# humanlongevity/tredparse

Hardware: NVIDIA B200
Metric: loci genotyped/sec (higher is better)
Workload: dtype int16 (SW, DPX s16x2) / f64 (likelihood)

## Files before the change

### tredparse_b200/csrc/sw_family.cu

```cuda
#include "internal.cuh"
#include "sw_sweep.cuh"
#include <type_traits>
#include <algorithm>
#include <vector>

namespace {

constexpr int FAM_W2 = 16;
constexpr int FLANK = 18;
constexpr int CLASS_BOTH = 0, CLASS_FWD = 1, CLASS_RC = 2, NCLASS = 3;

struct FamilySmem {
    int8_t prefix[32], suffix[32], repeat[32];
    int Lp, Ls, P, U, clip;
};

struct ClassifyParams {
    const int8_t *rbuf; const int64_t *roff;
    const int32_t *order;
    const int32_t *grp_start;
    const int32_t *chunk_start;
    const int32_t *grp_perm;
    const tredsw_family *families;
    int ngroups;
// ... 76 lines not shown
        Fv[C] = __viaddmax_s16x2(Fv[C], mge2, HOUT);                                          \
    }

constexpr int STAB_PAD = 20;

__host__ __device__ constexpr int strip_units(int P) { return P >= 12 ? 1 : 12 / P; }
__host__ __device__ constexpr int instance_period(int P) { return P == 6 ? 3 : P; }

template <int NC, int PER, bool HAS_IN, bool HAS_OUT, bool HOOK>
__device__ __forceinline__ void strip_pass(const uint32_t *stab, const uint8_t *codes, int lane, int m, int rows2,
                                           const uint32_t *bin, uint32_t *bout, const uint32_t *pot,
                                           uint32_t (&seg)[NC / PER], uint32_t (&mu)[NC / PER], uint32_t mgo2,
                                           uint32_t mge2, uint32_t one) {
    constexpr int K = NC / PER;
    static_assert(K * PER == NC, "strip = whole units");
    constexpr int NG = (NC + 3) / 4;
    uint32_t Hrow[NC], Fv[NC], pend[K];
#pragma unroll
    for (int c = 0; c < NC; ++c) { Hrow[c] = 0; Fv[c] = 0; }
#pragma unroll
    for (int u = 0; u < K; ++u) pend[u] = 0;
    uint32_t hin_prev = 0;
    auto code_at = [&](int j) { return j < m ? (int)codes[j * 32 + lane] : PAIR_GHOST; };
    auto row_of = [&](int code) { return reinterpret_cast<const uint4 *>(stab + code * STAB_PAD); };
    const uint4 *rowA = row_of(code_at(0)), *rowB = row_of(code_at(1));
    uint4 gA = rowA[0], gB = rowB[0];
    uint32_t bA = 0, bB = 0, pA = 0, pB = 0, bA2 = 0, bB2 = 0, pA2 = 0, pB2 = 0;
    const int j1 = min(2, rows2 - 2);
    if (HAS_IN) { bA = bin[lane]; bB = bin[32 + lane]; bA2 = bin[j1 * 32 + lane]; bB2 = bin[(j1 + 1) * 32 + lane]; }
    if (HOOK) { pA = pot[lane]; pB = pot[32 + lane]; pA2 = pot[j1 * 32 + lane]; pB2 = pot[(j1 + 1) * 32 + lane]; }
    int codeA2 = code_at(2), codeB2 = code_at(3);
    for (int j = 0; j < rows2; j += 2) {
        uint32_t hinA = 0, eA = 0, hinB = 0, eB = 0;
        if (HAS_IN) {
            hinA = sw_prmt(bA, 0, 0x4140); eA = sw_prmt(bA, 0, 0x4342);
            hinB = sw_prmt(bB, 0, 0x4140); eB = sw_prmt(bB, 0, 0x4342);
        }
        uint32_t potHA = 0, potEA = 0, potHB = 0, potEB = 0;
        if (HOOK) {
            potHA = sw_prmt(pA, 0, 0x9180); potEA = sw_prmt(pA, 0, 0xb3a2);
            potHB = sw_prmt(pB, 0, 0x9180); potEB = sw_prmt(pB, 0, 0xb3a2);
        }
        const int jn = min(j + 4, rows2 - 2);
        const uint4 *rowA2 = row_of(codeA2), *rowB2 = row_of(codeB2);
        uint32_t bA3 = 0, bB3 = 0, pA3 = 0, pB3 = 0;
        if (HAS_IN) { bA3 = bin[jn * 32 + lane]; bB3 = bin[(jn + 1) * 32 + lane]; }
        if (HOOK) { pA3 = pot[jn * 32 + lane]; pB3 = pot[(jn + 1) * 32 + lane]; }
        const int codeA3 = code_at(j + 4), codeB3 = code_at(j + 5);
        uint32_t sA[NG * 4], sB[NG * 4];
        sA[0] = gA.x; sA[1] = gA.y; sA[2] = gA.z; sA[3] = gA.w;
        sB[0] = gB.x; sB[1] = gB.y; sB[2] = gB.z; sB[3] = gB.w;
        uint32_t hdA = hin_prev, hdB = hinA;
        hin_prev = hinB;
        uint32_t hA = 0, hB = 0;
#pragma unroll
        for (int s = 0; s <= NC; ++s) {
            if ((s & 3) == 0 && s / 4 + 1 < NG) {
                const uint4 a = rowA[s / 4 + 1];
                sA[s + 4] = a.x; sA[s + 5] = a.y; sA[s + 6] = a.z; sA[s + 7] = a.w;
            }
            if (s >= 1 && ((s - 1) & 3) == 0 && (s - 1) / 4 + 1 < NG) {
                const uint4 b = rowB[(s - 1) / 4 + 1];
                sB[s + 3] = b.x; sB[s + 4] = b.y; sB[s + 5] = b.z; sB[s + 6] = b.w;
            }
            if (s == NC - 4 || (NC < 4 && s == 0)) { gA = rowA2[0]; gB = rowB2[0]; }
            if (s < NC) {
                PACKED_CELL(hdA, eA, sA[s], s, hA)
                const int u = s / PER, i = s % PER;
                if (i == 0) pend[u] = hA; else seg[u] = __vimax3_s16x2(seg[u], pend[u], hA);
                if (HOOK && i == PER - 1) {
                    mu[u] = __viaddmax_s16x2(hdA, potHA, mu[u]);
                    mu[u] = __viaddmax_s16x2(eA, potEA, mu[u]);
                }
                if (HAS_OUT && s == NC - 1) bout[j * 32 + lane] = sw_prmt(hA, eA, 0x6420);
            }
            if (s >= 1) {
                PACKED_CELL(hdB, eB, sB[s - 1], s - 1, hB)
                const int u = (s - 1) / PER, i = (s - 1) % PER;
                if (i == PER - 1) seg[u] = __vimax3_s16x2(seg[u], pend[u], hB); else pend[u] = hB;
                if (HOOK && i == PER - 1) {
                    mu[u] = __viaddmax_s16x2(hdB, potHB, mu[u]);
                    mu[u] = __viaddmax_s16x2(eB, potEB, mu[u]);
                }
                if (HAS_OUT && s - 1 == NC - 1) bout[(j + 1) * 32 + lane] = sw_prmt(hB, eB, 0x6420);
            }
        }
        rowA = rowA2; rowB = rowB2; codeA2 = codeA3; codeB2 = codeB3;
        bA = bA2; bB = bB2; bA2 = bA3; bB2 = bB3; pA = pA2; pB = pB2; pA2 = pA3; pB2 = pB3;
    }
}

template <int NC>
__device__ __forceinline__ void suffix_pass(const uint32_t *stab, const uint8_t *codes, int lane, int m, int rows2,
                                            uint32_t *pot, uint32_t &fresh, uint32_t mgo2, uint32_t mge2) {
    constexpr int NG = (NC + 3) / 4;
    uint32_t Grow[NC], Fv[NC];
#pragma unroll
    for (int c = 0; c < NC; ++c) { Grow[c] = 0; Fv[c] = 0; }
    auto code_at = [&](int r) { const int j = rows2 - 1 - r; return (j >= 0 && j < m) ? (int)codes[j * 32 + lane] : PAIR_GHOST; };
    auto row_of = [&](int code) { return reinterpret_cast<const uint4 *>(stab + code * STAB_PAD); };
    uint32_t f0 = 0, f1 = 0;
#define SUFFIX_CELL(GD, E, S, C, GOUT)                                                        \
    {                                                                                         \
        const uint32_t t_ = __vmaxs2(E, Fv[C]);                                               \
        const uint32_t gh_ = __viaddmax_s16x2_relu(t_, mgo2, GD);   \
        GD = Grow[C];                                                                         \
        GOUT = __vadd2(gh_, S);                                                               \
        Grow[C] = GOUT;                                                                       \
        E = __viaddmax_s16x2(E, mge2, gh_);                                                   \
        Fv[C] = __viaddmax_s16x2(Fv[C], mge2, gh_);                                           \
    }
    for (int r = 0; r < rows2; r += 2) {
        const uint4 *rowA = row_of(code_at(r)), *rowB = row_of(code_at(r + 1));
        uint32_t sA[NG * 4], sB[NG * 4];
#pragma unroll
        for (int g = 0; g < NG; ++g) {
            const uint4 a = rowA[g], b = rowB[g];
            sA[4 * g] = a.x; sA[4 * g + 1] = a.y; sA[4 * g + 2] = a.z; sA[4 * g + 3] = a.w;
            sB[4 * g] = b.x; sB[4 * g + 1] = b.y; sB[4 * g + 2] = b.z; sB[4 * g + 3] = b.w;
        }
        uint32_t gdA = 0, gdB = 0, eA = 0, eB = 0, gA = 0, gB = 0;
#pragma unroll
        for (int s = 0; s <= NC; ++s) {
            if (s < NC) { SUFFIX_CELL(gdA, eA, sA[s], s, gA) f0 = __vmaxs2(f0, gA); }
            if (s >= 1) { SUFFIX_CELL(gdB, eB, sB[s - 1], s - 1, gB) f1 = __vmaxs2(f1, gB); }
        }
        const int jA = rows2 - 1 - r, jB = jA - 1;
        pot[jA * 32 + lane] = jA < m ? sw_prmt(gA, __vadd2(eA, mgo2), 0x6420) : 0x80808080u;
        pot[jB * 32 + lane] = jB < m ? sw_prmt(gB, __vadd2(eB, mgo2), 0x6420) : 0x80808080u;
    }
#undef SUFFIX_CELL
    fresh = __vimax3_s16x2(f0, f1, 0u);
}

template <int NROWS>
__device__ __forceinline__ void build_stab(uint32_t *stab, const SwLut *lut, int lane, int ncols,
                                           const uint32_t *colsel ,
                                           uint32_t bias2 = 0u ) {
    static_assert(NROWS == NPAIR || NROWS == 6, "rows by pair code or by single code");
    for (int i = lane; i < NROWS * STAB_PAD; i += 32) {
        const int q = i / STAB_PAD, c = i % STAB_PAD;
        const int qa = NROWS == NPAIR ? q / 6 : q, qb = NROWS == NPAIR ? q % 6 : q;
        uint32_t v = 0u;
        if (c < ncols) {
            const uint32_t lo = sw_prmt(lut->w0[qa], lut->w1[qa], colsel[c]), hi = sw_prmt(lut->w0[qb], lut->w1[qb], colsel[c]);
            v = __vadd2(sw_prmt(lo, hi, 0x7610), bias2);
        }
        stab[i] = v;
    }
}

template <int NC, int PER, bool CAPTURE, class RowCode>
__device__ __forceinline__ void strip_locate(const uint32_t *stab, RowCode row_code, int rows2,
                                             const uint32_t *bin, uint32_t *bout, int kstar,
                                             uint32_t (&colkey)[NC], uint32_t mgo2, uint32_t mge2, uint32_t one) {
    constexpr int NG = (NC + 3) / 4;
    uint32_t Hrow[NC], Fv[NC];
#pragma unroll
    for (int c = 0; c < NC; ++c) { Hrow[c] = 0; Fv[c] = 0; colkey[c] = 0; }
    uint32_t hin_prev = 0;
    auto row_of = [&](int code) { return reinterpret_cast<const uint4 *>(stab + code * STAB_PAD); };
    uint32_t bA = bin[0], bB = bin[32];
    constexpr int KU = CAPTURE ? NC / PER : 1;
    uint32_t kmask[KU];
#pragma unroll
    for (int k = 0; k < KU; ++k) kmask[k] = (CAPTURE && k == kstar) ? 0xffffffffu : 0u;
    for (int j = 0; j < rows2; j += 2) {
        uint32_t capHA = 0, capEA = 0, capHB = 0, capEB = 0;
        const uint32_t hinA = sw_prmt(bA, 0, 0x4140), hinB = sw_prmt(bB, 0, 0x4140);
        uint32_t eA = sw_prmt(bA, 0, 0x4342), eB = sw_prmt(bB, 0, 0x4342);
        const int jn = min(j + 2, rows2 - 2);
        bA = bin[jn * 32]; bB = bin[(jn + 1) * 32];
        const uint4 *rowA = row_of(row_code(j)), *rowB = row_of(row_code(j + 1));
        uint32_t sA[NG * 4], sB[NG * 4];
#pragma unroll
        for (int g = 0; g < NG; ++g) {
            const uint4 a = rowA[g], b = rowB[g];
            sA[4 * g] = a.x; sA[4 * g + 1] = a.y; sA[4 * g + 2] = a.z; sA[4 * g + 3] = a.w;
            sB[4 * g] = b.x; sB[4 * g + 1] = b.y; sB[4 * g + 2] = b.z; sB[4 * g + 3] = b.w;
        }
        const uint32_t rcA = 0x00010001u * (uint32_t)(255 - j), rcB = rcA - 0x00010001u;
        uint32_t hdA = hin_prev, hdB = hinA;
        hin_prev = hinB;
        uint32_t hA = 0, hB = 0, keyA_prev = 0;
#pragma unroll
        for (int s = 0; s <= NC; ++s) {
            uint32_t keyA = 0;
            if (s < NC) {
                PACKED_CELL(hdA, eA, sA[s], s, hA)
                keyA = hA * 256u + rcA;
                if (CAPTURE && s % PER == PER - 1) { capHA |= hA & kmask[s / PER]; capEA |= eA & kmask[s / PER]; }
            }
            if (s >= 1) {
                PACKED_CELL(hdB, eB, sB[s - 1], s - 1, hB)
                const uint32_t keyB = hB * 256u + rcB;
                colkey[s - 1] = __vimax3_u16x2(colkey[s - 1], keyA_prev, keyB);
                if (CAPTURE && (s - 1) % PER == PER - 1) { capHB |= hB & kmask[(s - 1) / PER]; capEB |= eB & kmask[(s - 1) / PER]; }
            }
            keyA_prev = keyA;
        }
        if (CAPTURE) { bout[j * 32] = sw_prmt(capHA, capEA, 0x6420); bout[(j + 1) * 32] = sw_prmt(capHB, capEB, 0x6420); }
    }
}

template <int P>
__device__ __noinline__ void locate_packed(const FamilySmem &F, const SwLut *lut, uint32_t *stab, uint32_t *stab2,
                                           uint32_t *colsel, bool &suffix_table_ready, const uint8_t *codes, int lane,
                                           int m, int m_warp, uint32_t *bnd, const uint32_t *gbnd, int R, int go, int ge,
                                           uint32_t one, int G, int cs, int u, int u_main, int half, int sa, int sb,
                                           int *end_ref, int *end_read, unsigned long long &cells) {
    constexpr int K = strip_units(P);
    constexpr int NC = P * K;
    const uint32_t mgo2 = (uint32_t)((-go) & 0xffff) | ((uint32_t)((-go) & 0xffff) << 16);
    const uint32_t mge2 = (uint32_t)((-ge) & 0xffff) | ((uint32_t)((-ge) & 0xffff) << 16);
    const uint32_t go2 = (uint32_t)go * 0x00010001u;
    const int rows2 = (m_warp + 1) & ~1;
    const int su = G * (u_main > 0 ? u_main : u) - 1;
    const int tstar = su / K, kstar = su % K;
    const int sh = half ? 16 : 0;
    int found_col = -1, found_row = 0;
    {
        {
            const uint32_t *src = gbnd + (size_t)tstar * R * 32 + lane;
            for (int j = 0; j < rows2; ++j) bnd[j * 32 + lane] = src[j * 32];
        }
        uint32_t colkey[NC];
        auto pair_row = [&](int j) { return j < m ? (int)codes[j * 32 + lane] : PAIR_GHOST; };
        strip_locate<NC, P, true>(stab, pair_row, rows2, bnd + lane, bnd + lane, u_main > 0 ? -1 : kstar, colkey,
                                  mgo2, mge2, one);
        if (u_main > 0) {
#pragma unroll
            for (int c = NC - 1; c >= 0; --c) {
                const uint32_t k16 = (colkey[c] >> sh) & 0xffffu;
                if (c / P <= kstar && c / P > kstar - G && (int)(k16 >> 8) == cs) { found_col = FLANK + (tstar * K) * P + c; found_row = 255 - (int)(k16 & 0xffu); }
            }
        }
    }
    __syncwarp();
    cells += (unsigned long long)m * 2ull * (unsigned long long)NC;
    if (__any_sync(0xffffffffu, u_main <= 0 && cs < 0x7fff)) {
        if (!suffix_table_ready) {
            if (lane < FLANK) colsel[lane] = sel2(suf_base(F, sa, lane), suf_base(F, sb, lane));
            __syncwarp();
            build_stab<6>(stab2, lut, lane, FLANK, colsel, go2);
            __syncwarp();
            suffix_table_ready = true;
        }
        uint32_t colkey[FLANK];
        auto own_row = [&](int j) { return j < m ? pair_half(codes[j * 32 + lane], half) : SW_CODE_GHOST; };
        strip_locate<FLANK, FLANK, false>(stab2, own_row, rows2, bnd + lane, nullptr, 0, colkey, mgo2, mge2, one);
        if (u_main <= 0) {
#pragma unroll
            for (int c = FLANK - 1; c >= 0; --c) {
                const uint32_t k16 = (colkey[c] >> sh) & 0xffffu;
                if ((int)(k16 >> 8) == cs) { found_col = FLANK + u * F.P + c; found_row = 255 - (int)(k16 & 0xffu); }
            }
        }
        __syncwarp();
        cells += (unsigned long long)m * 2ull * (unsigned long long)FLANK;
    }
    *end_ref = found_col; *end_read = found_row;
}

template <int P>
__device__ __noinline__ void phase1_packed(const FamilySmem &F, const SwLut *lut, uint32_t *stab, uint32_t *colsel,
                                           const uint8_t *codes, int lane, int m, int m_warp, uint32_t *pot,
                                           uint32_t *gbnd, int R, uint8_t *scores, uint8_t *runs, int go, int ge,
                                           uint32_t one, int G, int sa, int sb, unsigned long long &cells) {
    constexpr int K = strip_units(P);
    constexpr int NC = P * K;
    static_assert(NC <= STAB_PAD && FLANK <= STAB_PAD, "strip wider than the score table");
    const uint32_t mgo2 = (uint32_t)((-go) & 0xffff) | ((uint32_t)((-go) & 0xffff) << 16);
    const uint32_t mge2 = (uint32_t)((-ge) & 0xffff) | ((uint32_t)((-ge) & 0xffff) << 16);
    const uint32_t go2 = (uint32_t)go * 0x00010001u;
    const int rows2 = (m_warp + 1) & ~1;
    if (lane < FLANK) colsel[lane] = sel2(suf_base(F, sa, FLANK - 1 - lane), suf_base(F, sb, FLANK - 1 - lane));
    __syncwarp();
    build_stab<NPAIR>(stab, lut, lane, FLANK, colsel);
    __syncwarp();
    uint32_t fresh = 0;
    suffix_pass<FLANK>(stab, codes, lane, m, rows2, pot, fresh, mgo2, mge2);
    __syncwarp();
    if (lane < FLANK) colsel[lane] = sel2(pre_base(F, sa, lane), pre_base(F, sb, lane));
    __syncwarp();
    build_stab<NPAIR>(stab, lut, lane, FLANK, colsel, go2);
    __syncwarp();
    uint32_t run;
    {
        uint32_t seg0[1] = {0u}, mu0[1] = {0u};
        strip_pass<FLANK, FLANK, false, true, false>(stab, codes, lane, m, rows2, nullptr, gbnd, pot, seg0, mu0, mgo2, mge2, one);
        run = seg0[0];
    }
    __syncwarp();
    for (int c = lane; c < NC; c += 32) colsel[c] = sel2(rep_base(F, sa, c % F.P), rep_base(F, sb, c % F.P));
    __syncwarp();
    build_stab<NPAIR>(stab, lut, lane, NC, colsel, go2);
    __syncwarp();
    int nstrips = 0;
    for (int u0 = 0; u0 < F.U * G; u0 += K, ++nstrips) {
        uint32_t seg[K], mu[K];
#pragma unroll
        for (int u = 0; u < K; ++u) { seg[u] = 0; mu[u] = 0; }
        strip_pass<NC, P, true, true, true>(stab, codes, lane, m, rows2, gbnd + (size_t)nstrips * R * 32,
                                            gbnd + (size_t)(nstrips + 1) * R * 32, pot, seg, mu, mgo2, mge2, one);
#pragma unroll
        for (int u = 0; u < K; ++u) {
            run = __vmaxs2(run, seg[u]);
            const int su = u0 + u + 1;
            if (su % G == 0 && su <= F.U * G) {
                const int ur = su / G - 1;
                const uint32_t best = __vimax3_s16x2(run, mu[u], fresh);
                scores[(2 * ur + 0) * 32 + lane] = (uint8_t)(best & 0xffu);
                scores[(2 * ur + 1) * 32 + lane] = (uint8_t)((best >> 16) & 0xffu);
                runs[(2 * ur + 0) * 32 + lane] = (uint8_t)(run & 0xffu);
                runs[(2 * ur + 1) * 32 + lane] = (uint8_t)((run >> 16) & 0xffu);
            }
        }
    }
    cells += (unsigned long long)m * 2ull * (unsigned long long)(2 * FLANK + nstrips * NC);
}

template <bool FAST>
__global__ void __launch_bounds__(32) classify_kernel(ClassifyParams p) {
    extern __shared__ __align__(16) unsigned char smem_raw[];
    __shared__ SwLut lut;
    __shared__ FamilySmem F;
    __shared__ __align__(16) uint32_t stab[NPAIR * STAB_PAD], stab2[6 * STAB_PAD];
    __shared__ uint32_t colsel[STAB_PAD];
    typedef typename std::conditional<FAST, uint8_t, uint16_t>::type score_t;
    const int lane = threadIdx.x;
    const int R = p.max_rows + 2;
    uint32_t *bnd = reinterpret_cast<uint32_t *>(smem_raw);
    uint8_t *codes = reinterpret_cast<uint8_t *>(bnd + (size_t)R * 32);
    unsigned char *slot = reinterpret_cast<unsigned char *>(p.score_buf) + (size_t)blockIdx.x * (2 * p.max_u) * 32 * sizeof(uint16_t);
    score_t *scores = reinterpret_cast<score_t *>(slot);
    uint8_t *runs = slot + (size_t)(2 * p.max_u) * 32;
    uint32_t *pot = FAST ? bnd : p.pot_buf + (size_t)blockIdx.x * R * 32;
    uint32_t *gbnd = p.gbnd_buf + (size_t)blockIdx.x * (p.nslots + 1) * R * 32;
    const uint32_t one = p.one;
    sw_build_lut(&lut, c_fmat25, lane, 32);
    const int nitems = p.chunk_start[p.ngroups];
    unsigned long long alg = 0, cells1 = 0, cells2 = 0;
    unsigned nal = 0;

    for (;;) {
        __syncwarp();
        int item = 0;
        if (lane == 0) item = atomicAdd(p.counter + (FAST ? 1 : 0), 1);
        item = __shfl_sync(0xffffffffu, item, 0);
        if (item >= nitems) break;
        int lo = 0, hi = p.ngroups;
        while (hi - lo > 1) {
            int mid = (lo + hi) >> 1;
            if (p.chunk_start[mid] <= item) lo = mid; else hi = mid;
        }
        const int grp = p.grp_perm[lo], f = grp / NCLASS, cls = grp % NCLASS;
        {
            const tredsw_family &g = p.families[f];
            F.prefix[lane] = g.prefix[lane]; F.suffix[lane] = g.suffix[lane]; F.repeat[lane] = g.repeat[lane];
            if (lane == 0) { F.Lp = g.prefix_len; F.Ls = g.suffix_len; F.P = g.period; F.U = g.max_units; F.clip = g.clip; }
        }
        __syncwarp();
        const bool fast_shape = p.allow_fast && (F.Lp == FLANK && F.Ls == FLANK && F.P >= 1 && F.P <= 12);
        if (fast_shape != FAST) continue;

        const bool pair = FAST && cls != CLASS_BOTH;
        const int sa = cls == CLASS_RC ? 1 : 0, sb = cls == CLASS_FWD ? 0 : 1;
        const int idx0 = p.grp_start[grp] + (pair ? 64 * (item - p.chunk_start[lo]) + 2 * lane : 32 * (item - p.chunk_start[lo]) + lane);
        int r0 = -1, r1 = -1, m0 = 0, m1 = 0;
        const bool valid0 = idx0 < p.grp_start[grp + 1], valid1 = pair && idx0 + 1 < p.grp_start[grp + 1];
        if (valid0) { r0 = p.order[idx0]; m0 = (int)(p.roff[r0 + 1] - p.roff[r0]); }
        if (valid1) { r1 = p.order[idx0 + 1]; m1 = (int)(p.roff[r1 + 1] - p.roff[r1]); }
        const bool too_long0 = m0 > p.max_rows, too_long1 = m1 > p.max_rows;
        if (too_long0) m0 = 0;
        if (too_long1) m1 = 0;
        auto clampc = [](int c) { return (c < 0 || c > 4) ? 4 : c; };
        const int m_lane = max(m0, m1);
        if (!pair) {
            if (m0 > 0) for_each_base(p.rbuf + p.roff[r0], m0, [&](int j, int c) { codes[j * 32 + lane] = (uint8_t)((FAST ? 7 : 1) * clampc(c)); });
        } else {
            if (m0 > 0) for_each_base(p.rbuf + p.roff[r0], m0, [&](int j, int c) { codes[j * 32 + lane] = (uint8_t)(6 * clampc(c) + SW_CODE_GHOST); });
            for (int j = m0; j < m_lane; ++j) codes[j * 32 + lane] = (uint8_t)PAIR_GHOST;
            if (m1 > 0) for_each_base(p.rbuf + p.roff[r1], m1, [&](int j, int c) { codes[j * 32 + lane] += (uint8_t)(clampc(c) - SW_CODE_GHOST); });
        }
        const int m_warp = __reduce_max_sync(0xffffffffu, m_lane);
        __syncwarp();

        if constexpr (!FAST) {
            phase1_generic(F, &lut, codes, lane, m0, m_warp, bnd, scores, p.go, p.ge, cells1);
        } else {
            switch (instance_period(F.P)) {
#define PCASE(PP) case PP: phase1_packed<PP>(F, &lut, stab, colsel, codes, lane, m_lane, m_warp, pot, gbnd, R, scores, runs, p.go, p.ge, one, F.P / PP, sa, sb, cells1); break;
                PCASE(1) PCASE(2) PCASE(3) PCASE(4) PCASE(5) PCASE(7) PCASE(8) PCASE(9) PCASE(10) PCASE(11) PCASE(12)
#undef PCASE
            }
        }
        __syncwarp();

        bool suffix_table_ready = false;
        for (int h = 0; h < (pair ? 2 : 1); ++h) {
            const bool valid = h ? valid1 : valid0, too_long = h ? too_long1 : too_long0;
            const int r = h ? r1 : r0, m = h ? m1 : m0;
            const int own_strand = h ? sb : sa;
            int tag = TREDSW_TAG_NONE, best_u = 0, best_score = -1, rb = -1, re = -1, qb = -1, qe = -1, best_rank = -1;
            const bool active = valid && m > 0;
            auto pick = [&](int last_score, int last_rank, int &cs, int &cr) {
                cs = -1; cr = -1;
                if (!active) return;
                for (int rank = 0; rank < 2 * F.U; ++rank) {
                    if (pair && (rank & 1) != own_strand) continue;
                    const int sc = scores[(pair ? (rank & ~1) | h : rank) * 32 + lane];
                    const int n = F.Lp + F.Ls + F.P * (rank / 2 + 1);
                    const int min_len = min(m, n) / 2;
                    if (sc < max(min_len, 30)) continue;
                    if (sc > last_score || (sc == last_score && rank <= last_rank)) continue;
                    if (sc > cs) { cs = sc; cr = rank; }
                }
            };
            int cs, cr;
            pick(0x7fffffff, -1, cs, cr);
            const int max_units_eff = F.clip ? (m + F.P - 1) / F.P : F.U;
            auto own_code = [&](int j) { return FAST ? pair_half(codes[j * 32 + lane], h) : (int)codes[j * 32 + lane]; };
            while (__any_sync(0xffffffffu, cr >= 0)) {
                const bool pending = cr >= 0;
                const int u = pending ? cr / 2 + 1 : 1, s = pending ? (cr & 1) : 0;
                const int half = pair ? h : s;
                int fast_end_ref = -1, fast_end_read = 0;
                if constexpr (FAST) {
                    if (FLANK * p.match < 30) {
                        int u_main = 0;
                        if (pending) for (int k = 1; k <= u; ++k) if ((int)runs[(2 * (k - 1) + half) * 32 + lane] == cs) { u_main = k; break; }
                        switch (instance_period(F.P)) {
#define PCASE(PP) case PP: locate_packed<PP>(F, &lut, stab, stab2, colsel, suffix_table_ready, codes, lane, m, m_warp, bnd, gbnd, R, p.go, p.ge, one, F.P / PP, pending ? cs : 0x7fff, u, u_main, half, sa, sb, &fast_end_ref, &fast_end_read, cells2); break;
                            PCASE(1) PCASE(2) PCASE(3) PCASE(4) PCASE(5) PCASE(7) PCASE(8) PCASE(9) PCASE(10) PCASE(11) PCASE(12)
#undef PCASE
                        }
                        if (!pending) fast_end_ref = -1;
                    }
                }
                if (pending) {
                    const int n = F.Lp + F.Ls + F.P * u;
                    auto cc_f = [&](int i) { return fam_code(F, u, s, n, i); };
                    int end_ref = fast_end_ref, end_read = fast_end_read;
                    if (end_ref < 0) {
                        const int drift = sw_max_drift(cs, m, n, p.match, p.go, p.ge);
                        const int need = (cs + p.match - 1) / p.match;
                        sw_sweep<FAM_W2, 1, false>(m, m, n, own_code, cc_f, &lut, bnd + lane, 32, p.go, p.ge, cs, &end_ref, &end_read,
                                                   nullptr, -(m - need) - drift, (n - need) + drift, &cells2);
                    }
                    bool settled = false;
                    if (end_ref >= 0) {
                        const int rdrift = sw_max_drift(cs, end_read + 1, end_ref + 1, p.match, p.go, p.ge);
                        int ci = -1, rj = 0;
                        if (rdrift == 0) {
                            const int lim = min(end_read, end_ref) + 1;
                            int hs = 0;
                            for (int k = 0; k < lim; ++k) {
                                const int qc = own_code(end_read - k);
                                const int sc = (int)sw_prmt(lut.w0[qc], lut.w1[qc], sw_sel32(fam_code(F, u, s, n, end_ref - k)));
                                hs = max(0, hs + sc);
                                if (hs == cs) { ci = rj = k; break; }
                            }
                            cells2 += (unsigned long long)lim;
                        }
                        if (ci < 0) {
                            auto rc_r = [&](int j) { return own_code(end_read - j); };
                            auto cc_r = [&](int i) { return fam_code(F, u, s, n, end_ref - i); };
                            sw_sweep<FAM_W2, 1, false>(end_read + 1, end_read + 1, end_ref + 1, rc_r, cc_r, &lut, bnd + lane, 32,
                                                       p.go, p.ge, cs, &ci, &rj, nullptr, -rdrift, rdrift, &cells2);
                        }
                        const int c_rb = end_ref - ci, c_qb = end_read - rj;
                        const int t = sw_classify(cs, c_rb, end_ref, c_qb, end_read, m, n, u, F.P, max_units_eff);
                        if (t != TREDSW_TAG_NONE) {
                            tag = t; best_u = u; best_score = cs; rb = c_rb; re = end_ref; qb = c_qb; qe = end_read;
                            best_rank = cr;
                            settled = true;
                        }
                    }
                    if (settled) cr = -1;
                    else { const int ls = cs, lr = cr; pick(ls, lr, cs, cr); }
                }
                __syncwarp();
            }
            if (valid) {
                int32_t *o = p.out + (int64_t)r * 8;
                o[0] = too_long ? -1 : tag; o[1] = best_u; o[2] = best_score; o[3] = rb; o[4] = re; o[5] = qb; o[6] = qe;
                o[7] = best_rank;
            }
            if (p.stats && active) {
                unsigned long long sum_n = 0;
                for (int u = 1; u <= F.U; ++u) sum_n += 2ull * (unsigned long long)(F.Lp + F.Ls + F.P * u);
                alg += (unsigned long long)m * sum_n;
                nal += (unsigned)(2 * F.U);
            }
        }
    }
    if (p.stats) {
        unsigned long long c1 = cells1, c2 = cells2, na = nal;
        for (int d = 16; d > 0; d >>= 1) {
            alg += __shfl_down_sync(0xffffffffu, alg, d);
            c1 += __shfl_down_sync(0xffffffffu, c1, d);
            c2 += __shfl_down_sync(0xffffffffu, c2, d);
            na += __shfl_down_sync(0xffffffffu, na, d);
        }
        if (lane == 0) {
            atomicAdd(&p.stats[0], alg); atomicAdd(&p.stats[1], c1); atomicAdd(&p.stats[2], c2);
            atomicAdd(&p.stats[3], na);
        }
    }
}

struct QgramInfo {
    int q;
    int min_score;
    int pair;
};
constexpr int QTAB_WORDS = 256;

__global__ void prefilter_kernel(const int8_t *rbuf, const int64_t *roff, int nreads, const int32_t *read_family,
                                 int nfam, const tredsw_family *families, const uint32_t *qtab, const QgramInfo *qinfo,
                                 int b_minus, int32_t *eff_group, unsigned long long *stats) {
    const int r = blockIdx.x * blockDim.x + threadIdx.x;
    unsigned long long alg = 0; unsigned nal = 0;
    if (r < nreads) {
        int f = read_family[r], cls = CLASS_BOTH;
        if (f < 0 || f >= nfam) f = -1;
        if (f >= 0 && qinfo[f].q > 0) {
            const int q = qinfo[f].q;
            const uint32_t mask = (1u << (2 * q)) - 1u;
            const uint32_t *tab = qtab + (size_t)f * QTAB_WORDS;
            const int8_t *s = rbuf + roff[r];
            const int m = (int)(roff[r + 1] - roff[r]);
            uint32_t code = 0; int run = 0, nN = 0, hf = 0, hr = 0;
            for_each_base(s, m, [&](int, int c) {
                if (c < 0 || c > 3) { ++nN; run = 0; return; }
                code = ((code << 2) | (uint32_t)c) & mask;
                if (++run >= q) {
                    const uint32_t e = (tab[code >> 4] >> ((code & 15u) * 2u)) & 3u;
                    hf += e & 1u; hr += e >> 1;
                }
            });
            const int thr = qinfo[f].min_score - (q - 1) * (nN + 1);
            if (hf < thr && hr < thr) {
                if (stats) {
                    const tredsw_family &g = families[f];
                    unsigned long long sum_n = 0;
                    for (int u = 1; u <= g.max_units; ++u) sum_n += 2ull * (unsigned long long)(g.prefix_len + g.suffix_len + g.period * u);
                    alg = (unsigned long long)m * sum_n; nal = 2u * (unsigned)g.max_units;
                }
                f = -2;
            } else if (qinfo[f].pair && (hf < thr || hr < thr)) {
                cls = hf >= thr ? CLASS_FWD : CLASS_RC;
            }
        }
        eff_group[r] = f >= 0 ? f * NCLASS + cls : f;
    }
    if (stats) {
        for (int d = 16; d > 0; d >>= 1) { alg += __shfl_down_sync(0xffffffffu, alg, d); nal += __shfl_down_sync(0xffffffffu, nal, d); }
        if ((threadIdx.x & 31) == 0 && alg) { atomicAdd(&stats[0], alg); atomicAdd(&stats[3], (unsigned long long)nal); }
    }
}

__global__ void fam_count_kernel(const int32_t *read_group, int nreads, int ngroups, int32_t *count) {
    const int r = blockIdx.x * blockDim.x + threadIdx.x;
    int f = r < nreads ? read_group[r] : -1;
    if (f >= ngroups) f = -1;
    const unsigned peers = __match_any_sync(0xffffffffu, f);
    if (f >= 0 && (threadIdx.x & 31) == __ffs(peers) - 1) atomicAdd(&count[f], __popc(peers));
}
__global__ void fam_scan_kernel(const int32_t *count, int ngroups, const int32_t *perm, int32_t *grp_start,
                                int32_t *chunk_start, int32_t *cursor) {
    if (threadIdx.x == 0 && blockIdx.x == 0) {
        int a = 0, b = 0;
        for (int g = 0; g < ngroups; ++g) { grp_start[g] = a; cursor[g] = a; a += count[g]; }
        grp_start[ngroups] = a;
        for (int i = 0; i < ngroups; ++i) {
            const int per = perm[i] % NCLASS == CLASS_BOTH ? 32 : 64;
            chunk_start[i] = b; b += (count[perm[i]] + per - 1) / per;
        }
        chunk_start[ngroups] = b;
    }
}
__global__ void fam_scatter_kernel(const int32_t *read_group, int nreads, int ngroups, int32_t *cursor,
                                   int32_t *order, int32_t *out) {
    const int r = blockIdx.x * blockDim.x + threadIdx.x;
    const int lane = threadIdx.x & 31;
    int f = r < nreads ? read_group[r] : -1;
    if (f >= ngroups) f = -1;
    const unsigned peers = __match_any_sync(0xffffffffu, f);
    const int leader = __ffs(peers) - 1;
    int base = 0;
    if (f >= 0 && lane == leader) base = atomicAdd(&cursor[f], __popc(peers));
    base = __shfl_sync(0xffffffffu, base, leader);
    if (r < nreads) {
        if (f >= 0) order[base + __popc(peers & ((1u << lane) - 1u))] = r;
        else if (f == -2) {
            int32_t *o = out + (int64_t)r * 8; o[0] = TREDSW_TAG_NONE; o[1] = 0; o[2] = o[3] = o[4] = o[5] = o[6] = o[7] = -1;
        } else { int32_t *o = out + (int64_t)r * 8; o[0] = -1; o[1] = o[2] = o[3] = o[4] = o[5] = o[6] = o[7] = -1; }
    }
}

template <bool FAST>
int launch_classify(tredsw_ctx *ctx, const ClassifyParams &p, int nctas, size_t smem) {
    classify_kernel<FAST><<<nctas, 32, smem, ctx->stream>>>(p);
    CUDA_TRY(cudaGetLastError());
    ctx->launches += 1;
    return TREDSW_OK;
}

int classify_static_smem(size_t *out) {
    cudaFuncAttributes fa{}, ga{};
    CUDA_TRY(cudaFuncGetAttributes(&fa, classify_kernel<true>));
    CUDA_TRY(cudaFuncGetAttributes(&ga, classify_kernel<false>));
    *out = std::max(fa.sharedSizeBytes, ga.sharedSizeBytes);
    return TREDSW_OK;
}

int persistent_ctas(tredsw_ctx *ctx, size_t smem, size_t static_smem, bool need_fast, bool need_generic, int *out) {
    int a = 0, b = 0;
    if (smem + static_smem > 48 * 1024) {
        CUDA_TRY(cudaFuncSetAttribute(classify_kernel<true>, cudaFuncAttributeMaxDynamicSharedMemorySize, (int)smem));
        CUDA_TRY(cudaFuncSetAttribute(classify_kernel<false>, cudaFuncAttributeMaxDynamicSharedMemorySize, (int)smem));
    }
    if (need_fast) CUDA_TRY(cudaOccupancyMaxActiveBlocksPerMultiprocessor(&a, classify_kernel<true>, 32, smem));
    if (need_generic) CUDA_TRY(cudaOccupancyMaxActiveBlocksPerMultiprocessor(&b, classify_kernel<false>, 32, smem));
    int per_sm = need_fast ? a : b;
    static const int env_cap = [] { const char *e = getenv("TREDSW_CTAS_PER_SM"); return e ? atoi(e) : 0; }();
    const int cap = env_cap > 0 ? env_cap : 8;
    if (per_sm > cap) per_sm = cap;
    if (per_sm < 1) per_sm = 1;
    static const int env_free = [] { const char *e = getenv("TREDSW_FREE_SLOTS"); return e ? atoi(e) : -1; }();
    int free_slots = env_free >= 0 ? env_free : 0;
    if (free_slots > per_sm * ctx->sm_count / 2) free_slots = per_sm * ctx->sm_count / 2;
    *out = per_sm * ctx->sm_count - free_slots;
    return TREDSW_OK;
}

}

int tredsw_internal_classify(tredsw_ctx *ctx, const int8_t *d_rbuf, const int64_t *d_roff, int nreads,
                             const int32_t *d_read_family, const tredsw_family *d_families,
                             const tredsw_family *h_families, int nfamilies, int max_m,
                             const int8_t *mat25, int gap_open, int gap_extend, int32_t *d_work, int32_t *d_out,
                             unsigned long long *d_stats) {
    int max_u = 0, nslots = 1; bool need_fast = false, need_generic = false; int max_match = 0;
// ... 203 lines not shown
```

Baseline: 1.792 million.

## Locate both read halves in one packed strip sweep instead of two passes

The phase-2 end-locating loop is restructured so that both reads of a pair (or both strands) are processed together: the packed strip sweep carries one candidate per 16-bit half, with per-half capture masks and per-half boundary columns merged via byte permute. This replaces the sequential per-half loop and its duplicated packed sweeps, and drops the separate single-code suffix table by rebuilding the pair-code table in place when needed. The cost is toggling the shared table between repeat and suffix contents on each iteration, plus more per-read state held in registers.

```diff
diff --git a/tredparse_b200/csrc/sw_family.cu b/tredparse_b200/csrc/sw_family.cu
--- a/tredparse_b200/csrc/sw_family.cu
+++ b/tredparse_b200/csrc/sw_family.cu
@@ -252,7 +252,7 @@
 
 template <int NC, int PER, bool CAPTURE, class RowCode>
 __device__ __forceinline__ void strip_locate(const uint32_t *stab, RowCode row_code, int rows2,
-                                             const uint32_t *bin, uint32_t *bout, int kstar,
+                                             const uint32_t *bin, uint32_t *bout, int kstar_a, int kstar_b,
                                              uint32_t (&colkey)[NC], uint32_t mgo2, uint32_t mge2, uint32_t one) {
     constexpr int NG = (NC + 3) / 4;
     uint32_t Hrow[NC], Fv[NC];
@@ -264,7 +264,7 @@
     constexpr int KU = CAPTURE ? NC / PER : 1;
     uint32_t kmask[KU];
 #pragma unroll
-    for (int k = 0; k < KU; ++k) kmask[k] = (CAPTURE && k == kstar) ? 0xffffffffu : 0u;
+    for (int k = 0; k < KU; ++k) kmask[k] = (CAPTURE && k == kstar_a ? 0x0000ffffu : 0u) | (CAPTURE && k == kstar_b ? 0xffff0000u : 0u);
     for (int j = 0; j < rows2; j += 2) {
         uint32_t capHA = 0, capEA = 0, capHB = 0, capEB = 0;
         const uint32_t hinA = sw_prmt(bA, 0, 0x4140), hinB = sw_prmt(bB, 0, 0x4140);
@@ -304,10 +304,10 @@
 }
 
 template <int P>
-__device__ __noinline__ void locate_packed(const FamilySmem &F, const SwLut *lut, uint32_t *stab, uint32_t *stab2,
-                                           uint32_t *colsel, bool &suffix_table_ready, const uint8_t *codes, int lane,
-                                           int m, int m_warp, uint32_t *bnd, const uint32_t *gbnd, int R, int go, int ge,
-                                           uint32_t one, int G, int cs, int u, int u_main, int half, int sa, int sb,
+__device__ __noinline__ void locate_packed(const FamilySmem &F, const SwLut *lut, uint32_t *stab, uint32_t *colsel,
+                                           bool &stab_suffix, const uint8_t *codes, int lane, int m_lane, int m_warp,
+                                           uint32_t *bnd, const uint32_t *gbnd, int R, int go, int ge, uint32_t one, int G,
+                                           int cs0, int u0, int um0, int cs1, int u1, int um1, int sa, int sb,
                                            int *end_ref, int *end_read, unsigned long long &cells) {
     constexpr int K = strip_units(P);
     constexpr int NC = P * K;
@@ -315,51 +315,66 @@
     const uint32_t mge2 = (uint32_t)((-ge) & 0xffff) | ((uint32_t)((-ge) & 0xffff) << 16);
     const uint32_t go2 = (uint32_t)go * 0x00010001u;
     const int rows2 = (m_warp + 1) & ~1;
-    const int su = G * (u_main > 0 ? u_main : u) - 1;
-    const int tstar = su / K, kstar = su % K;
-    const int sh = half ? 16 : 0;
-    int found_col = -1, found_row = 0;
+    const int cs[2] = {cs0, cs1}, u[2] = {u0, u1}, um[2] = {um0, um1};
+    int tstar[2], kstar[2];
+#pragma unroll
+    for (int h = 0; h < 2; ++h) {
+        const int su = G * (um[h] > 0 ? um[h] : u[h]) - 1;
+        tstar[h] = su / K; kstar[h] = su % K;
+        end_ref[h] = -1; end_read[h] = 0;
+    }
+    if (stab_suffix) {
+        for (int c = lane; c < NC; c += 32) colsel[c] = sel2(rep_base(F, sa, c % F.P), rep_base(F, sb, c % F.P));
+        __syncwarp();
+        build_stab<NPAIR>(stab, lut, lane, NC, colsel, go2);
+        __syncwarp();
+        stab_suffix = false;
+    }
+    auto pair_row = [&](int j) { return j < m_lane ? (int)codes[j * 32 + lane] : PAIR_GHOST; };
     {
         {
-            const uint32_t *src = gbnd + (size_t)tstar * R * 32 + lane;
-            for (int j = 0; j < rows2; ++j) bnd[j * 32 + lane] = src[j * 32];
+            const uint32_t *src0 = gbnd + (size_t)tstar[0] * R * 32 + lane, *src1 = gbnd + (size_t)tstar[1] * R * 32 + lane;
+            for (int j = 0; j < rows2; ++j) bnd[j * 32 + lane] = sw_prmt(src0[j * 32], src1[j * 32], 0x7250);
         }
         uint32_t colkey[NC];
-        auto pair_row = [&](int j) { return j < m ? (int)codes[j * 32 + lane] : PAIR_GHOST; };
-        strip_locate<NC, P, true>(stab, pair_row, rows2, bnd + lane, bnd + lane, u_main > 0 ? -1 : kstar, colkey,
-                                  mgo2, mge2, one);
-        if (u_main > 0) {
-#pragma unroll
-            for (int c = NC - 1; c >= 0; --c) {
-                const uint32_t k16 = (colkey[c] >> sh) & 0xffffu;
-                if (c / P <= kstar && c / P > kstar - G && (int)(k16 >> 8) == cs) { found_col = FLANK + (tstar * K) * P + c; found_row = 255 - (int)(k16 & 0xffu); }
+        strip_locate<NC, P, true>(stab, pair_row, rows2, bnd + lane, bnd + lane, um[0] > 0 ? -1 : kstar[0],
+                                  um[1] > 0 ? -1 : kstar[1], colkey, mgo2, mge2, one);
+#pragma unroll
+        for (int h = 0; h < 2; ++h) {
+            if (um[h] > 0) {
+#pragma unroll
+                for (int c = NC - 1; c >= 0; --c) {
+                    const uint32_t k16 = (colkey[c] >> (16 * h)) & 0xffffu;
+                    if (c / P <= kstar[h] && c / P > kstar[h] - G && (int)(k16 >> 8) == cs[h]) {
+                        end_ref[h] = FLANK + (tstar[h] * K) * P + c; end_read[h] = 255 - (int)(k16 & 0xffu);
+                    }
+                }
             }
         }
     }
     __syncwarp();
-    cells += (unsigned long long)m * 2ull * (unsigned long long)NC;
-    if (__any_sync(0xffffffffu, u_main <= 0 && cs < 0x7fff)) {
-        if (!suffix_table_ready) {
-            if (lane < FLANK) colsel[lane] = sel2(suf_base(F, sa, lane), suf_base(F, sb, lane));
-            __syncwarp();
-            build_stab<6>(stab2, lut, lane, FLANK, colsel, go2);
-            __syncwarp();
-            suffix_table_ready = true;
-        }
+    cells += (unsigned long long)m_lane * 2ull * (unsigned long long)NC;
+    if (__any_sync(0xffffffffu, (um[0] <= 0 && cs[0] < 0x7fff) || (um[1] <= 0 && cs[1] < 0x7fff))) {
+        if (lane < FLANK) colsel[lane] = sel2(suf_base(F, sa, lane), suf_base(F, sb, lane));
+        __syncwarp();
+        build_stab<NPAIR>(stab, lut, lane, FLANK, colsel, go2);
+        __syncwarp();
+        stab_suffix = true;
         uint32_t colkey[FLANK];
-        auto own_row = [&](int j) { return j < m ? pair_half(codes[j * 32 + lane], half) : SW_CODE_GHOST; };
-        strip_locate<FLANK, FLANK, false>(stab2, own_row, rows2, bnd + lane, nullptr, 0, colkey, mgo2, mge2, one);
-        if (u_main <= 0) {
-#pragma unroll
-            for (int c = FLANK - 1; c >= 0; --c) {
-                const uint32_t k16 = (colkey[c] >> sh) & 0xffffu;
-                if ((int)(k16 >> 8) == cs) { found_col = FLANK + u * F.P + c; found_row = 255 - (int)(k16 & 0xffu); }
+        strip_locate<FLANK, FLANK, false>(stab, pair_row, rows2, bnd + lane, nullptr, 0, 0, colkey, mgo2, mge2, one);
+#pragma unroll
+        for (int h = 0; h < 2; ++h) {
+            if (um[h] <= 0) {
+#pragma unroll
+                for (int c = FLANK - 1; c >= 0; --c) {
+                    const uint32_t k16 = (colkey[c] >> (16 * h)) & 0xffffu;
+                    if ((int)(k16 >> 8) == cs[h]) { end_ref[h] = FLANK + u[h] * F.P + c; end_read[h] = 255 - (int)(k16 & 0xffu); }
+                }
             }
         }
         __syncwarp();
-        cells += (unsigned long long)m * 2ull * (unsigned long long)FLANK;
-    }
-    *end_ref = found_col; *end_read = found_row;
+        cells += (unsigned long long)m_lane * 2ull * (unsigned long long)FLANK;
+    }
 }
 
 template <int P>
@@ -425,7 +440,7 @@
     extern __shared__ __align__(16) unsigned char smem_raw[];
     __shared__ SwLut lut;
     __shared__ FamilySmem F;
-    __shared__ __align__(16) uint32_t stab[NPAIR * STAB_PAD], stab2[6 * STAB_PAD];
+    __shared__ __align__(16) uint32_t stab[NPAIR * STAB_PAD];
     __shared__ uint32_t colsel[STAB_PAD];
     typedef typename std::conditional<FAST, uint8_t, uint16_t>::type score_t;
     const int lane = threadIdx.x;
@@ -497,60 +512,79 @@
         }
         __syncwarp();
 
-        bool suffix_table_ready = false;
-        for (int h = 0; h < (pair ? 2 : 1); ++h) {
-            const bool valid = h ? valid1 : valid0, too_long = h ? too_long1 : too_long0;
-            const int r = h ? r1 : r0, m = h ? m1 : m0;
-            const int own_strand = h ? sb : sa;
-            int tag = TREDSW_TAG_NONE, best_u = 0, best_score = -1, rb = -1, re = -1, qb = -1, qe = -1, best_rank = -1;
-            const bool active = valid && m > 0;
-            auto pick = [&](int last_score, int last_rank, int &cs, int &cr) {
-                cs = -1; cr = -1;
-                if (!active) return;
+        const int nrd = pair ? 2 : 1;
+        const bool valid[2] = {valid0, valid1}, too_long[2] = {too_long0, too_long1};
+        const int rid[2] = {r0, r1}, mr[2] = {m0, m1};
+        int tag[2], best_u[2], best_score[2], rb[2], re[2], qb[2], qe[2], best_rank[2], cs[2], cr[2];
+        auto pick = [&](int i, int last_score, int last_rank) {
+            int bs = -1, br = -1;
+            if (valid[i] && mr[i] > 0) {
                 for (int rank = 0; rank < 2 * F.U; ++rank) {
-                    if (pair && (rank & 1) != own_strand) continue;
-                    const int sc = scores[(pair ? (rank & ~1) | h : rank) * 32 + lane];
+                    if (pair && (rank & 1) != (i ? sb : sa)) continue;
+                    const int sc = scores[(pair ? (rank & ~1) | i : rank) * 32 + lane];
                     const int n = F.Lp + F.Ls + F.P * (rank / 2 + 1);
-                    const int min_len = min(m, n) / 2;
+                    const int min_len = min(mr[i], n) / 2;
                     if (sc < max(min_len, 30)) continue;
                     if (sc > last_score || (sc == last_score && rank <= last_rank)) continue;
-                    if (sc > cs) { cs = sc; cr = rank; }
+                    if (sc > bs) { bs = sc; br = rank; }
                 }
-            };
-            int cs, cr;
-            pick(0x7fffffff, -1, cs, cr);
-            const int max_units_eff = F.clip ? (m + F.P - 1) / F.P : F.U;
-            auto own_code = [&](int j) { return FAST ? pair_half(codes[j * 32 + lane], h) : (int)codes[j * 32 + lane]; };
-            while (__any_sync(0xffffffffu, cr >= 0)) {
-                const bool pending = cr >= 0;
-                const int u = pending ? cr / 2 + 1 : 1, s = pending ? (cr & 1) : 0;
-                const int half = pair ? h : s;
-                int fast_end_ref = -1, fast_end_read = 0;
-                if constexpr (FAST) {
-                    if (FLANK * p.match < 30) {
-                        int u_main = 0;
-                        if (pending) for (int k = 1; k <= u; ++k) if ((int)runs[(2 * (k - 1) + half) * 32 + lane] == cs) { u_main = k; break; }
-                        switch (instance_period(F.P)) {
-#define PCASE(PP) case PP: locate_packed<PP>(F, &lut, stab, stab2, colsel, suffix_table_ready, codes, lane, m, m_warp, bnd, gbnd, R, p.go, p.ge, one, F.P / PP, pending ? cs : 0x7fff, u, u_main, half, sa, sb, &fast_end_ref, &fast_end_read, cells2); break;
-                            PCASE(1) PCASE(2) PCASE(3) PCASE(4) PCASE(5) PCASE(7) PCASE(8) PCASE(9) PCASE(10) PCASE(11) PCASE(12)
+            }
+            cs[i] = bs; cr[i] = br;
+        };
+#pragma unroll
+        for (int i = 0; i < 2; ++i) {
+            tag[i] = TREDSW_TAG_NONE; best_u[i] = 0; best_score[i] = -1; rb[i] = re[i] = qb[i] = qe[i] = best_rank[i] = -1;
+            cs[i] = -1; cr[i] = -1;
+            if (i < nrd) pick(i, 0x7fffffff, -1);
+        }
+        bool stab_suffix = false;
+        while (__any_sync(0xffffffffu, cr[0] >= 0 || cr[1] >= 0)) {
+            int fast_end_ref[2] = {-1, -1}, fast_end_read[2] = {0, 0};
+            if constexpr (FAST) {
+                if (FLANK * p.match < 30) {
+                    int hcs[2] = {0x7fff, 0x7fff}, hu[2] = {1, 1}, hum[2] = {0, 0};
+#pragma unroll
+                    for (int i = 0; i < 2; ++i) {
+                        if (i < nrd && cr[i] >= 0) {
+                            const int h = pair ? i : (cr[i] & 1), u = cr[i] / 2 + 1;
+                            hcs[h] = cs[i]; hu[h] = u;
+                            for (int k = 1; k <= u; ++k) if ((int)runs[(2 * (k - 1) + h) * 32 + lane] == cs[i]) { hum[h] = k; break; }
+                        }
+                    }
+                    int er[2], ed[2];
+                    switch (instance_period(F.P)) {
+#define PCASE(PP) case PP: locate_packed<PP>(F, &lut, stab, colsel, stab_suffix, codes, lane, m_lane, m_warp, bnd, gbnd, R, p.go, p.ge, one, F.P / PP, hcs[0], hu[0], hum[0], hcs[1], hu[1], hum[1], sa, sb, er, ed, cells2); break;
+                        PCASE(1) PCASE(2) PCASE(3) PCASE(4) PCASE(5) PCASE(7) PCASE(8) PCASE(9) PCASE(10) PCASE(11) PCASE(12)
 #undef PCASE
+                    }
+#pragma unroll
+                    for (int i = 0; i < 2; ++i) {
+                        if (i < nrd && cr[i] >= 0) {
+                            const int h = pair ? i : (cr[i] & 1);
+                            fast_end_ref[i] = er[h]; fast_end_read[i] = ed[h];
                         }
-                        if (!pending) fast_end_ref = -1;
                     }
                 }
-                if (pending) {
+            }
+#pragma unroll
+            for (int i = 0; i < 2; ++i) {
+                if (i < nrd && cr[i] >= 0) {
+                    const int m = mr[i], u = cr[i] / 2 + 1, s = cr[i] & 1;
+                    const int half = pair ? i : s;
                     const int n = F.Lp + F.Ls + F.P * u;
-                    auto cc_f = [&](int i) { return fam_code(F, u, s, n, i); };
-                    int end_ref = fast_end_ref, end_read = fast_end_read;
+                    const int max_units_eff = F.clip ? (m + F.P - 1) / F.P : F.U;
+                    auto own_code = [&](int j) { return FAST ? pair_half(codes[j * 32 + lane], half) : (int)codes[j * 32 + lane]; };
+                    auto cc_f = [&](int c) { return fam_code(F, u, s, n, c); };
+                    int end_ref = fast_end_ref[i], end_read = fast_end_read[i];
                     if (end_ref < 0) {
-                        const int drift = sw_max_drift(cs, m, n, p.match, p.go, p.ge);
-                        const int need = (cs + p.match - 1) / p.match;
-                        sw_sweep<FAM_W2, 1, false>(m, m, n, own_code, cc_f, &lut, bnd + lane, 32, p.go, p.ge, cs, &end_ref, &end_read,
-                                                   nullptr, -(m - need) - drift, (n - need) + drift, &cells2);
+                        const int drift = sw_max_drift(cs[i], m, n, p.match, p.go, p.ge);
+                        const int need = (cs[i] + p.match - 1) / p.match;
+                        sw_sweep<FAM_W2, 1, false>(m, m, n, own_code, cc_f, &lut, bnd + lane, 32, p.go, p.ge, cs[i], &end_ref,
+                                                   &end_read, nullptr, -(m - need) - drift, (n - need) + drift, &cells2);
                     }
                     bool settled = false;
                     if (end_ref >= 0) {
-                        const int rdrift = sw_max_drift(cs, end_read + 1, end_ref + 1, p.match, p.go, p.ge);
+                        const int rdrift = sw_max_drift(cs[i], end_read + 1, end_ref + 1, p.match, p.go, p.ge);
                         int ci = -1, rj = 0;
                         if (rdrift == 0) {
                             const int lim = min(end_read, end_ref) + 1;
@@ -559,38 +593,41 @@
                                 const int qc = own_code(end_read - k);
                                 const int sc = (int)sw_prmt(lut.w0[qc], lut.w1[qc], sw_sel32(fam_code(F, u, s, n, end_ref - k)));
                                 hs = max(0, hs + sc);
-                                if (hs == cs) { ci = rj = k; break; }
+                                if (hs == cs[i]) { ci = rj = k; break; }
                             }
                             cells2 += (unsigned long long)lim;
                         }
                         if (ci < 0) {
                             auto rc_r = [&](int j) { return own_code(end_read - j); };
-                            auto cc_r = [&](int i) { return fam_code(F, u, s, n, end_ref - i); };
+                            auto cc_r = [&](int c) { return fam_code(F, u, s, n, end_ref - c); };
                             sw_sweep<FAM_W2, 1, false>(end_read + 1, end_read + 1, end_ref + 1, rc_r, cc_r, &lut, bnd + lane, 32,
-                                                       p.go, p.ge, cs, &ci, &rj, nullptr, -rdrift, rdrift, &cells2);
+                                                       p.go, p.ge, cs[i], &ci, &rj, nullptr, -rdrift, rdrift, &cells2);
                         }
                         const int c_rb = end_ref - ci, c_qb = end_read - rj;
-                        const int t = sw_classify(cs, c_rb, end_ref, c_qb, end_read, m, n, u, F.P, max_units_eff);
+                        const int t = sw_classify(cs[i], c_rb, end_ref, c_qb, end_read, m, n, u, F.P, max_units_eff);
                         if (t != TREDSW_TAG_NONE) {
-                            tag = t; best_u = u; best_score = cs; rb = c_rb; re = end_ref; qb = c_qb; qe = end_read;
-                            best_rank = cr;
+                            tag[i] = t; best_u[i] = u; best_score[i] = cs[i]; rb[i] = c_rb; re[i] = end_ref; qb[i] = c_qb;
+                            qe[i] = end_read; best_rank[i] = cr[i];
                             settled = true;
                         }
                     }
-                    if (settled) cr = -1;
-                    else { const int ls = cs, lr = cr; pick(ls, lr, cs, cr); }
+                    if (settled) cr[i] = -1;
+                    else pick(i, cs[i], cr[i]);
                 }
-                __syncwarp();
-            }
-            if (valid) {
-                int32_t *o = p.out + (int64_t)r * 8;
-                o[0] = too_long ? -1 : tag; o[1] = best_u; o[2] = best_score; o[3] = rb; o[4] = re; o[5] = qb; o[6] = qe;
-                o[7] = best_rank;
-            }
-            if (p.stats && active) {
+            }
+            __syncwarp();
+        }
+#pragma unroll
+        for (int i = 0; i < 2; ++i) {
+            if (i < nrd && valid[i]) {
+                int32_t *o = p.out + (int64_t)rid[i] * 8;
+                o[0] = too_long[i] ? -1 : tag[i]; o[1] = best_u[i]; o[2] = best_score[i]; o[3] = rb[i]; o[4] = re[i];
+                o[5] = qb[i]; o[6] = qe[i]; o[7] = best_rank[i];
+            }
+            if (p.stats && i < nrd && valid[i] && mr[i] > 0) {
                 unsigned long long sum_n = 0;
                 for (int u = 1; u <= F.U; ++u) sum_n += 2ull * (unsigned long long)(F.Lp + F.Ls + F.P * u);
-                alg += (unsigned long long)m * sum_n;
+                alg += (unsigned long long)mr[i] * sum_n;
                 nal += (unsigned)(2 * F.U);
             }
         }
```

New measurement: 1.946 million, median of 6. +8.6%, better.
